# hku-mars/ImMesh

Measured on AMD Instinct MI355X. Metric: scans/sec (reg+mesh), 100k-pt scan into 10M-voxel map, higher is better.
Workload: dtype f64

## Files before the change

### immesh_amd/csrc/c_api.cpp

```cpp
#include "host_ctx.hpp"
#include "imu_host.hpp"
#include <cmath>
#include <new>

#define RP_ABORTED 1
static thread_local std::string g_create_error;
thread_local KProf* g_kprof = nullptr;



extern "C" {

void immesh_default_config(immesh_config* c) {
    std::memset(c, 0, sizeof(*c));
    c->voxel_size = 0.5; c->max_layer = 2;
    for (int i = 0; i < 5; i++) c->layer_init[i] = 5;
    c->max_points_size = 100; c->planer_threshold = 0.01; c->dept_err = 0.02; c->beam_err = 0.05; c->calib_laser = 0;
    c->sigma_num = 3.0; c->max_iter = 4;
    c->extR[0] = c->extR[4] = c->extR[8] = 1.0;
    c->extT[0] = 0.04165; c->extT[1] = 0.02326; c->extT[2] = -0.0284;
    c->mesh_min_spacing = 0.1; c->mesh_voxel = 0.4; c->mesh_region = 10.0; c->mesh_append_budget = 10000;
}

const char* immesh_create_error(void) { return g_create_error.c_str(); }
// ... 413 lines not shown

struct IngestOpts {
    int mode = 0;
    hipEvent_t after_point_var = nullptr;
    const ScanParams* spd = nullptr;
    const float* d_raw = nullptr; float* world = nullptr; int n_raw = 0;
    bool defer_tail = false;
    bool prep_done = false;
};
static int map_ingest_device(immesh_ctx* c, const float* d_pts, int64_t n, const imh::State& st, const IngestOpts& o) {
    ScanParams sp;
    make_scan_params(c, st, st.cov, sp);
    hipStream_t s = c->stream;
    if (o.mode == 0) {
        if (!o.prep_done) {
            if (c->tail_deferred) { launch_map_update_tail(s, c->map, c->d_counters_host); c->tail_deferred = false; }
            c->map.upd_seq++;
            c->map.touched = c->d_touched;
            launch_point_var(s, c->map, sp, o.spd, d_pts, (int)n, 3, o.mode, c->d_ptdata, c->d_key_a, c->d_slot, c->d_idx_a, o.d_raw, o.world, o.n_raw);
            if (o.world) { c->ev_inputs_cur = mesh_record_ready(c); c->inputs_seq = 0; }
            else if (o.after_point_var) { HIPCHK(c, hipEventRecord(o.after_point_var, s)); c->ev_inputs_cur = o.after_point_var; c->inputs_seq = 0; }
        }
        launch_replay_lists(s, c->map, c->d_idx_a, c->d_key_a, c->d_ptdata, (int)n, c->d_stats, c->d_counters_host, c->d_idx_b, c->d_idx_c, c->d_slot_s, c->reg_dbg, !o.defer_tail,
                            o.prep_done ? (unsigned long long*)(c->d_epi + 2) : nullptr, o.prep_done ? c->d_epi_flag_host : nullptr, c->epi_seq, c->knobs.fused_wgs, c->knobs.list_div);
        c->tail_deferred = o.defer_tail;
        return 0;
    }
    launch_point_var(s, c->map, sp, nullptr, d_pts, (int)n, 3, o.mode, c->d_ptdata, c->d_key_a, c->d_slot, nullptr);
    launch_iota(s, c->d_idx_a, (int)n);
    sort_pairs_u32(s, c->d_sort_temp, c->sort_temp_bytes, c->d_slot, c->d_slot_s, c->d_idx_a, c->d_idx_c, (int)n, 32);
    launch_segment_heads(s, c->d_slot_s, (int)n, c->d_seg_start, c->d_nseg);
    launch_replay(s, c->map, c->d_slot_s, c->d_idx_c, c->d_ptdata, (int)n, c->d_seg_start, c->d_nseg, (int)n, o.mode, c->d_stats);
    HIPCHK(c, hipMemcpyAsync(c->h_counters, c->map.counters, 16 * sizeof(int32_t), hipMemcpyDeviceToHost, s));
    return 0;
}

static int map_ingest_entry(immesh_ctx* c, const float* pts, int64_t n, const double* state, int mode) {
    if (!c || !pts || n <= 0 || n > c->cap_scan || !state) { if (c) c->err = "bad arguments"; return IMMESH_E_INVAL; }
    (void)hipSetDevice(c->cfg.device);
    ProfBind _pb(c);
    if (mode == 0) c->ds_gate_ok = false;
    if (const int s_rc = settle(c)) return s_rc;
    const void* d_pts;
    int rc = resolve_input(c, pts, (size_t)n * 12, c->d_pts_down, &d_pts);
    if (rc) return rc;
    imh::State st;
    imh::load_state(state, st);
// ... 300 lines not shown
```

### immesh_amd/csrc/host_knobs.hpp

```cpp
#pragma once
#include <hip/hip_runtime.h>
#include <algorithm>
#include <cstdlib>
#include <cstring>
#include <string>

struct Knobs {
    bool debug = false;
    bool debug_waits = false;
    std::string trace_file;
    int split_general = -1;
    bool no_priority = false;
    int mesh_cus = 0;
    int rp_blocks = 0;
    bool rp_force_abort = false;
    bool match_seq = false;
    bool host_ekf = false;
    bool serial_safe = false;
    bool serial_order = false;
    bool ds_radix = false;
    bool ds_no_gate = false;
    bool no_graph = false;
    int split_mode = 2;
    int mesh_room = 0;
    bool no_pipeline = false;
    int tri_stream = 1;
    int fused_wgs = 768;
    int list_div = 0;
    int mesh_grid_div = 1;

    static Knobs from_env(int mesh_npar) {
        auto on = [](const char* name) { return getenv(name) != nullptr; };
        auto num = [](const char* name, int unset) { const char* e = getenv(name); return e ? atoi(e) : unset; };
        Knobs k;
        k.debug = on("IMMESH_DEBUG"); k.debug_waits = on("IMMESH_DEBUG_WAITS");
        if (const char* e = getenv("IMMESH_TRACE_FILE")) k.trace_file = e;
        if (on("IMMESH_SPLIT_GENERAL")) k.split_general = num("IMMESH_SPLIT_GENERAL", 0);
        k.no_priority = on("IMMESH_NO_PRIORITY");
        k.mesh_cus = num("IMMESH_MESH_CUS", 0); if (k.mesh_cus < 8 || k.mesh_cus >= 1024) k.mesh_cus = 0;
        if (on("IMMESH_RP_BLOCKS")) k.rp_blocks = std::max(1, num("IMMESH_RP_BLOCKS", 0));
        k.rp_force_abort = on("IMMESH_RP_FORCE_ABORT"); k.match_seq = on("IMMESH_MATCH_SEQ"); k.host_ekf = on("IMMESH_HOST_EKF");
        k.serial_safe = on("IMMESH_SERIAL_SAFE"); k.serial_order = on("IMMESH_SERIAL_ORDER");
        k.ds_radix = on("IMMESH_DS_RADIX"); k.ds_no_gate = on("IMMESH_DS_NO_GATE");
        k.no_graph = on("IMMESH_NO_GRAPH");
        k.split_mode = on("IMMESH_NO_SPLIT") ? 0 : 2;
        if (on("IMMESH_SPLIT")) k.split_mode = num("IMMESH_SPLIT", 0) == 0 ? 0 : 1;
        if (on("IMMESH_MESH_ROOM")) k.mesh_room = std::min(std::max(num("IMMESH_MESH_ROOM", 0), 1), mesh_npar);
        k.no_pipeline = on("IMMESH_NO_PIPELINE");
        k.tri_stream = num("IMMESH_TRI_STREAM", 1);
        { const int v = num("IMMESH_FUSED_WGS", 0); k.fused_wgs = v >= 32 ? v : 768; }
        { const int v = num("IMMESH_LIST_DIV", 0); k.list_div = v >= 4 ? v : 0; }
        k.mesh_grid_div = std::max(1, num("IMMESH_MESH_GRID_DIV", 1));
        return k;
    }

    hipError_t make_stream(hipStream_t* s, int priority, bool maskable) const {
        if (!maskable || !mesh_cus) return hipStreamCreateWithPriority(s, hipStreamNonBlocking, priority);
        uint32_t mask[32];
        std::memset(mask, 0, sizeof(mask));
        for (int i = 0; i < mesh_cus; i++) mask[i >> 5] |= 1u << (i & 31);
        return hipExtStreamCreateWithCUMask(s, 32, mask);
    }
};
```

### immesh_amd/csrc/kernels.hpp

```cpp
#pragma once
#include <hip/hip_runtime.h>
#include <stdint.h>

struct RegMapDev;

struct ScanParams {
    double R[9], t[3];
    double extR[9], extT[3];
    double RextR[9];
    double rot_var[9], t_var[9];
    double dvar_beam;
    double dvar_calib;
    double sigma_num;
    float dept_err;
    int calib_laser;
    unsigned long long* dbg;
};

struct PlaneRecDev {
    long long key[3];
    int layer, path, is_plane, n_points, update_enable, new_points;
    float radius, min_eig, d, pad;
    double center[3], normal[3], plane_var[36];
};
// ... 37 lines not shown
};
static_assert(REG_OUT_COV + 18 * 18 == REG_OUT_PASSES && REG_OUT_TICKET == REG_OUT_DOUBLES - 1, "registration result block layout");

void launch_residual(hipStream_t s, const RegMapDev& m, const RegIterArgs& a, RegState* rs, const float* pts, int n, double* partials, unsigned int* done_counter,
                     double* out48, double* reg_out, double ticket, int8_t* o_match, int32_t* o_node, float* o_dis, double* o_rinv, double* o_normal);
#define RP_SLOT_DOUBLES (64 * 128 * 32)
#define RP_SLOT_SENTINEL 0x7FF8DEADBEEF0001ull
struct RpEpilogue {
    int enabled, n_raw;
    double* pt_data; unsigned long long* sort_key; uint32_t* slot_out; int32_t* pt_next;
    const float* raw; float* world;
};
#define RP_TAIL_WORD (63 * 128 * 32)
#define RP_ABORT_WORD (62 * 128 * 32)
void launch_residual_persistent(hipStream_t s, const RegMapDev& m, const RegIterArgs& a, RegState* rs, const float* pts, int n, double* slots, double* slots_next,
                                int32_t* host_counters, double* reg_out, double ticket, int8_t* o_match, int32_t* o_node, float* o_dis, double* o_rinv, double* o_normal,
                                const RpEpilogue& ep, int max_blocks);
int residual_persistent_resident_blocks(int device);
void launch_ekf_step(hipStream_t s, const RegIterArgs& a, RegState* rs, const double* sums48, double* reg_out, double ticket);
void launch_point_var(hipStream_t s, const RegMapDev& m, const ScanParams& sp, const ScanParams* spd, const float* pts, int n, int stride, int mode, double* pt_data,
                      unsigned long long* sort_key, uint32_t* slot, int32_t* pt_next, const float* raw_xyzi = nullptr, float* world_xyzi = nullptr, int n_raw = 0);
void launch_replay_lists(hipStream_t s, const RegMapDev& m, const int32_t* pt_next, const unsigned long long* sort_key, const double* pt_data, int n,
                         int64_t* stats, int32_t* host_counters, int32_t* big_idx, int32_t* big_order, uint32_t* general_list, unsigned long long* dbg, bool with_tail, unsigned long long* flag_dev, unsigned long long* flag_host, unsigned long long flag_seq,
                         int fused_wgs, int list_div_knob);
void launch_map_update_tail(hipStream_t s, const RegMapDev& m, int32_t* host_counters);
void launch_segment_heads(hipStream_t s, const uint32_t* sorted_slot, int n, int32_t* seg_start, int32_t* nseg);
void launch_replay(hipStream_t s, const RegMapDev& m, const uint32_t* sorted_slot, const int32_t* sorted_idx, const double* pt_data, int n,
                   const int32_t* seg_start, const int32_t* nseg, int max_segments, int mode, int64_t* stats);
void launch_dump_planes(hipStream_t s, const RegMapDev& m, PlaneRecDev* out, long long cap, unsigned long long* count);
void launch_fill_u64(hipStream_t s, unsigned long long* p, unsigned long long v, size_t n);
void launch_iota(hipStream_t s, int32_t* p, int n);
void launch_unpack_strided(hipStream_t s, const void* src, int n, int stride_bytes, int intensity_off_bytes, float* out);

void launch_ds_minmax(hipStream_t s, const float* pts, int n, int stride, float inv, int* mm);
void launch_ds_index(hipStream_t s, const float* pts, int n, int stride, float inv, const int* mm, unsigned long long* keys, int32_t* vals);
void launch_ds_heads(hipStream_t s, const unsigned long long* keys_sorted, int n, int32_t* flags);
void launch_ds_centroid(hipStream_t s, const float* pts, int n, int stride, const unsigned long long* keys_sorted, const int32_t* idx_sorted, const int32_t* rank,
                        float* out, int32_t* n_out);
void launch_decode_livox_count(hipStream_t s, const uint8_t* w, int n, int n_scans, int32_t* counted);
void launch_decode_livox_keep(hipStream_t s, const uint8_t* w, int n, int n_scans, int filter, double blind_sqr, const int32_t* valid_excl, int32_t* keep);
void launch_decode_livox_emit(hipStream_t s, const uint8_t* w, int n, const int32_t* keep, const int32_t* pos, float* out, int32_t* n_out);
void launch_decode_velodyne_keep(hipStream_t s, const uint8_t* d, int n, int step, int ox, int oy, int oz, float q_lo, float q_hi, int32_t* keep);
void launch_decode_velodyne_emit(hipStream_t s, const uint8_t* d, int n, int step, int ox, int oy, int oz, int oi, const int32_t* keep, const int32_t* pos, float* out,
                                 int32_t* n_out);
void launch_undistort_keys(hipStream_t s, const float* pts5, int n, uint32_t* key, int32_t* idx);
void launch_undistort(hipStream_t s, const float* pts5, const int32_t* order, int n, const double* poses, int n_poses, const double* fe, float* out_xyzi);
struct DsDyn { const float* pts; float* out; int32_t n, stride; float inv; int32_t pad; const int32_t* gate_word; int32_t gate_val, gate_pad; };
// ... 16 lines not shown
```

### immesh_amd/csrc/reg_kernels.hip

```cpp
#include <algorithm>
#include <cstdlib>
#include "regmap.hpp"
#include "kernels.hpp"
#include "prof.hpp"

using namespace imd;

struct PlaneRegs { double n[3], c[3], pv[21]; float d, radius; };
struct BestMatch { int node; int layer; double prob; bool ok; PlaneRegs P; };

IMD double plane_sigma(const double* pv, const double* J) {
    double tmp[6];
#pragma unroll
    for (int c = 0; c < 6; c++) {
        double s = 0;
#pragma unroll
        for (int r = 0; r < 6; r++) s += J[r] * pv[(r <= c) ? sym21_index(r, c) : sym21_index(c, r)];
        tmp[c] = s;
    }
    double sig = 0;
#pragma unroll
    for (int c = 0; c < 6; c++) sig += tmp[c] * J[c];
    return sig;
}
// ... 1305 lines not shown
        const double Umin[3] = {sel3(imin, f.U[0], f.U[1], f.U[2]), sel3(imin, f.U[3], f.U[4], f.U[5]), sel3(imin, f.U[6], f.U[7], f.U[8])};
        if (lane < 21) {
            double v = 0;
#pragma unroll
            for (int k = 0; k < 21; k++) if (lane == k) v = pv[k];
            nr.p_var[lane] = v;
        }
        if (lane == 0) {
            const double evmin = sel3(imin, f.ev[0], f.ev[1], f.ev[2]);
            const double evmax = sel3(f.imax, f.ev[0], f.ev[1], f.ev[2]);
#pragma unroll
            for (int k = 0; k < 3; k++) { nr.p_center[k] = f.c[k]; nr.p_normal[k] = Umin[k]; }
            nr.min_eig = (float)evmin;
            nr.radius = (float)sqrt(evmax);
            nr.d = (float)(-(Umin[0] * f.c[0] + Umin[1] * f.c[1] + Umin[2] * f.c[2]));
        }
    } else if (lane == 0) {
#pragma unroll
        for (int k = 0; k < 3; k++) { nr.p_center[k] = f.c[k]; nr.p_normal[k] = 0.0; }
        nr.radius = 0.f;
    }
}

__device__ __noinline__ bool wave_init_plane(const RegMapDev& m, int nd, int n, const WaveCtx& w) {
    __builtin_amdgcn_fence(__ATOMIC_ACQUIRE, "workgroup");
    if (w.lane == 0 && w.stats) { atomicAdd((unsigned long long*)&w.stats[0], 1ull); atomicAdd((unsigned long long*)&w.stats[1], (unsigned long long)n); }
    PlaneFit f;
    double pv[21];
    const int lane = w.lane;
    if (n <= 128) {
        double P0[9], P1[9];
#pragma unroll
        for (int k = 0; k < 9; k++) { P0[k] = 0; P1[k] = 0; }
        if (lane < n) { const double* q = node_point_ptr(m, nd, lane);
#pragma unroll
            for (int k = 0; k < 9; k++) P0[k] = q[k]; }
        if (lane + 64 < n) { const double* q = node_point_ptr(m, nd, lane + 64);
#pragma unroll
            for (int k = 0; k < 9; k++) P1[k] = q[k]; }
        auto fe = [&](auto&& fn) __attribute__((always_inline)) { if (lane < n) fn(P0); if (lane + 64 < n) fn(P1); };
        fit_eigen(fe, n, m.planer_threshold, f);
        if (f.planar) fit_plane_var(fe, n, f, pv);
    } else {
        auto fe = [&](auto&& fn) __attribute__((always_inline)) {
            for (int i = lane; i < n; i += 64) {
                const double* q = node_point_ptr(m, nd, i);
                double P[9];
#pragma unroll
                for (int k = 0; k < 9; k++) P[k] = q[k];
                fn(P);
            }
        };
        fit_eigen(fe, n, m.planer_threshold, f);
        if (f.planar) fit_plane_var(fe, n, f, pv);
    }
    fit_store(m.nodes[nd], f, pv, lane);
    return f.planar;
}

__device__ bool wave_push_point(const RegMapDev& m, int nd, int n, const double* src, const WaveCtx& w) {
    int ok = 1;
    if (w.lane == 0 && (n % IM_CHUNK_PTS) == 0) ok = node_ensure_chunk(m, nd, n / IM_CHUNK_PTS) ? 1 : 0;
    ok = __shfl(ok, 0, 64);
    if (!ok) return false;
    __builtin_amdgcn_fence(__ATOMIC_RELEASE, "workgroup");
    __builtin_amdgcn_fence(__ATOMIC_ACQUIRE, "workgroup");
    if (w.lane < IM_PT_DOUBLES) {
        double* dst = node_point_ptr(m, nd, n);
        dst[w.lane] = src[w.lane];
    }
    __builtin_amdgcn_fence(__ATOMIC_RELEASE, "workgroup");
    return true;
}

IMD int octant_of(const double* q, const double* center) {
    return 4 * (q[0] > center[0] ? 1 : 0) + 2 * (q[1] > center[1] ? 1 : 0) + (q[2] > center[2] ? 1 : 0);
}
IMD int make_child(const RegMapDev& m, int nd, int oct) {
    const float ql = m.nodes[nd].quarter;
    const int xyz[3] = {(oct >> 2) & 1, (oct >> 1) & 1, oct & 1};
    double c[3];
#pragma unroll
    for (int k = 0; k < 3; k++) c[k] = m.nodes[nd].center[k] + (double)((float)(2 * xyz[k] - 1) * ql);
    const int layer = m.nodes[nd].layer + 1;
    const int child = node_alloc(m, layer, c, ql / 2, m.nodes[nd].key, m.nodes[nd].path | (oct << (3 * (layer - 1))));
    m.nodes[nd].child[oct] = child;
    return child;
}

__device__ void wave_init_octo_tree(const RegMapDev& m, int node, int* stack, const WaveCtx& w) {
    int sp = 0;
    if (w.lane == 0) stack[0] = node;
    sp = 1;
    while (sp > 0) {
        __builtin_amdgcn_fence(__ATOMIC_ACQUIRE, "workgroup");
        const int nd = __shfl(stack[sp - 1], 0, 64);
        sp--;
        const int n = m.nodes[nd].npts;
        const bool planar = wave_init_plane(m, nd, n, w);
        const int layer = m.nodes[nd].layer;
        if (w.lane == 0) {
            const int f0 = m.nodes[nd].flags;
            int f = f0 | NF_INIT;
            f = planar ? (f | NF_PLANE) : (f & ~NF_PLANE);
            node_set_flags(m, w.root, nd, f0, f, w.shared);
            m.nodes[nd].newpts = 0;
        }
        if (planar || layer >= m.max_layer) continue;
        const double ctr[3] = {m.nodes[nd].center[0], m.nodes[nd].center[1], m.nodes[nd].center[2]};
        int child_id[8], child_n[8];
#pragma unroll
        for (int k = 0; k < 8; k++) { child_id[k] = m.nodes[nd].child[k]; child_n[k] = child_id[k] >= 0 ? m.nodes[child_id[k]].npts : 0; }
        for (int base = 0; base < n; base += 64) {
            const int i = base + w.lane;
            const double* q = (i < n) ? node_point_ptr(m, nd, i) : nullptr;
            const int oct = (i < n) ? octant_of(q, ctr) : -1;
#pragma unroll
            for (int k = 0; k < 8; k++) {
                const unsigned long long mask = __ballot(oct == k);
                if (mask == 0) continue;
                const int cnt = __popcll(mask);
                int cid = child_id[k];
// ... 15 lines not shown
#pragma unroll
                    for (int e = 0; e < IM_PT_DOUBLES; e++) dst[e] = q[e];
                }
                child_n[k] += cnt;
            }
        }
        __builtin_amdgcn_fence(__ATOMIC_RELEASE, "workgroup");
        if (w.lane == 0) {
#pragma unroll
            for (int k = 0; k < 8; k++)
                if (child_id[k] >= 0) { m.nodes[child_id[k]].npts = child_n[k]; m.nodes[child_id[k]].newpts = child_n[k]; }
            node_free_points(m, nd);
        }
#pragma unroll
        for (int k = 7; k >= 0; k--)
            if (child_id[k] >= 0 && child_n[k] > m.init_size[min(layer + 1, 4)]) {
                if (w.lane == 0) stack[sp] = child_id[k];
                sp++;
            }
        __builtin_amdgcn_fence(__ATOMIC_RELEASE, "workgroup");
    }
}

__device__ void wave_update_point(const RegMapDev& m, int root, const double* src, int* stack, const WaveCtx& w) {
    int nd = root;
    for (int depth = 0; depth < 8; depth++) {
        __builtin_amdgcn_fence(__ATOMIC_ACQUIRE, "workgroup");
        const int flags = m.nodes[nd].flags;
        const int layer = m.nodes[nd].layer;
        const int n = m.nodes[nd].npts;
        if (!(flags & NF_INIT)) {
            if (!wave_push_point(m, nd, n, src, w)) return;
            if (w.lane == 0) { m.nodes[nd].npts = n + 1; m.nodes[nd].newpts = m.nodes[nd].newpts + 1; }
            __builtin_amdgcn_fence(__ATOMIC_RELEASE, "workgroup");
            if (n + 1 > m.init_size[min(layer, 4)]) wave_init_octo_tree(m, nd, stack, w);
            return;
        }
        if (flags & NF_PLANE) {
            if (!(flags & NF_UPDATE_EN)) return;
            if (!wave_push_point(m, nd, n, src, w)) return;
            int newp = m.nodes[nd].newpts + 1;
            if (w.lane == 0) m.nodes[nd].npts = n + 1;
            __builtin_amdgcn_fence(__ATOMIC_RELEASE, "workgroup");
            if (newp > 5) {
                const bool planar = wave_init_plane(m, nd, n + 1, w);
                if (w.lane == 0) node_set_flags(m, w.root, nd, flags, planar ? (flags | NF_PLANE) : (flags & ~NF_PLANE), w.shared);
                newp = 0;
            }
            if (w.lane == 0) {
                m.nodes[nd].newpts = newp;
                if (n + 1 >= m.max_points_size) {
                    m.nodes[nd].flags = m.nodes[nd].flags & ~NF_UPDATE_EN;
                    node_free_points(m, nd);
                    m.nodes[nd].newpts = 0;
                }
            }
            __builtin_amdgcn_fence(__ATOMIC_RELEASE, "workgroup");
            return;
        }
        if (layer < m.max_layer) {
            int child;
            if (w.lane == 0) {
                if (n != 0) node_free_points(m, nd);
                const double ctr[3] = {m.nodes[nd].center[0], m.nodes[nd].center[1], m.nodes[nd].center[2]};
                const int oct = octant_of(src, ctr);
                child = m.nodes[nd].child[oct];
                if (child < 0) child = make_child(m, nd, oct);
            }
            __builtin_amdgcn_fence(__ATOMIC_RELEASE, "workgroup");
            child = __shfl(child, 0, 64);
            if (child < 0) return;
            nd = child;
            continue;
        }
        if (!(flags & NF_UPDATE_EN)) return;
        if (!wave_push_point(m, nd, n, src, w)) return;
        int newp = m.nodes[nd].newpts + 1;
        if (w.lane == 0) m.nodes[nd].npts = n + 1;
        __builtin_amdgcn_fence(__ATOMIC_RELEASE, "workgroup");
        if (newp > 5) {
            const bool planar = wave_init_plane(m, nd, n + 1, w);
            if (w.lane == 0) node_set_flags(m, w.root, nd, flags, planar ? (flags | NF_PLANE) : (flags & ~NF_PLANE), w.shared);
            newp = 0;
        }
        if (w.lane == 0) {
            m.nodes[nd].newpts = newp;
            if (n + 1 > IM_G_MAX_POINTS) { m.nodes[nd].flags = m.nodes[nd].flags & ~NF_UPDATE_EN; node_free_points(m, nd); }
        }
        __builtin_amdgcn_fence(__ATOMIC_RELEASE, "workgroup");
        return;
    }
}

__device__ int wave_replay_planar_root(const RegMapDev& m, const int root, const int* order, const int cnt, const double* __restrict__ pt_data, const WaveCtx& w) {
    NodeRec& nd = m.nodes[root];
    int flags = nd.flags;
    const int layer = nd.layer;
    int npts = nd.npts, newp = nd.newpts;
    const int want = NF_INIT | NF_PLANE | NF_UPDATE_EN;
    if (layer == 0 && (flags & want) == (NF_INIT | NF_PLANE)) return cnt;
    if ((flags & want) != want || layer != 0 || npts + cnt > IM_INLINE_CHUNKS * IM_CHUNK_PTS) return 0;
    int chunks[IM_INLINE_CHUNKS];
#pragma unroll
    for (int k = 0; k < IM_INLINE_CHUNKS; k++) chunks[k] = nd.chunks[k];
    auto chunk_of = [&](int ci) { int c = chunks[0];
#pragma unroll
        for (int k = 1; k < IM_INLINE_CHUNKS; k++) { const int ck = chunks[k]; c = (ci == k) ? ck : c; }
        return c; };
    double s1[3] = {0, 0, 0}, s2[3] = {0, 0, 0};
    const bool will_refit = newp + cnt > 5;
    if (will_refit) {
        for (int i = w.lane; i < npts; i += 64) {
            const double* q = m.chunk_data + ((size_t)chunk_of(i / IM_CHUNK_PTS) * IM_CHUNK_PTS + (i % IM_CHUNK_PTS)) * IM_PT_DOUBLES;
#pragma unroll
            for (int a = 0; a < 3; a++) { const double v = q[a]; s1[a] += v; s2[a] += v * v; }
        }
// ... 24 lines not shown
            if (c < 0) { write_header(); return j; }
#pragma unroll
            for (int k = 0; k < IM_INLINE_CHUNKS; k++) if (ci == k) chunks[k] = c;
        }
        const double pv = w.lane < IM_PT_DOUBLES ? src[w.lane] : 0.0;
        if (w.lane < IM_PT_DOUBLES) m.chunk_data[((size_t)chunk_of(ci) * IM_CHUNK_PTS + (npts % IM_CHUNK_PTS)) * IM_PT_DOUBLES + w.lane] = pv;
        if (will_refit) {
#pragma unroll
            for (int a = 0; a < 3; a++) { const double v = __shfl(pv, a, 64); s1[a] += v; s2[a] += v * v; }
        }
        npts++; newp++; header_dirty = true;
        if (newp > 5) {
            n_ref++; n_ref_pts += npts;
            const double dn = (double)npts;
            double vmin = 1e300, mag = 0;
#pragma unroll
            for (int a = 0; a < 3; a++) { const double mu = s1[a] / dn; const double v = s2[a] / dn - mu * mu; vmin = fmin(vmin, v); mag += s2[a] / dn; }
            const double err = 1e-7 + 1e-12 * mag;
            newp = 0;
            if (vmin + err < (double)m.planer_threshold) last_refit_n = npts;
            else {
                write_header();
                last_refit_n = 0;
                const bool planar = wave_init_plane(m, root, npts, wq);
                if (!planar) {
                    if (w.lane == 0) node_set_flags(m, w.root, root, flags, flags & ~NF_PLANE);
                    __builtin_amdgcn_fence(__ATOMIC_RELEASE, "workgroup");
                    flags &= ~NF_PLANE;
                    if (npts >= m.max_points_size) {
                        flags &= ~NF_UPDATE_EN;
                        write_header();
                        if (w.lane == 0) { node_free_points(m, root); nd.newpts = 0; }
                        __builtin_amdgcn_fence(__ATOMIC_RELEASE, "workgroup");
                        npts = 0; newp = 0;
                    }
                    j++;
                    break;
                }
            }
        }
        if (npts >= m.max_points_size) {
            if (last_refit_n) { write_header(); (void)wave_init_plane(m, root, last_refit_n, wq); last_refit_n = 0; }
            flags &= ~NF_UPDATE_EN;
            write_header();
            if (w.lane == 0) { node_free_points(m, root); nd.newpts = 0; }
            __builtin_amdgcn_fence(__ATOMIC_RELEASE, "workgroup");
            npts = 0; newp = 0;
            j++;
            break;
        }
    }
    if (header_dirty) write_header();
    if (last_refit_n) (void)wave_init_plane(m, root, last_refit_n, wq);
    if (w.lane == 0 && w.stats && n_ref) { atomicAdd((unsigned long long*)&w.stats[0], (unsigned long long)n_ref); atomicAdd((unsigned long long*)&w.stats[1], (unsigned long long)n_ref_pts); }
    return j;
}

__device__ int wave_replay_planar_node(const RegMapDev& m, const int node, const int* order, const int cnt, const double* __restrict__ pt_data, const WaveCtx& w) {
    NodeRec& nd = m.nodes[node];
    int flags = nd.flags;
    const int want = NF_INIT | NF_PLANE | NF_UPDATE_EN;
    if ((flags & want) == (NF_INIT | NF_PLANE)) return cnt;
    if ((flags & want) != want) return 0;
    int npts = nd.npts, newp = nd.newpts;
    double s1[3] = {0, 0, 0}, s2[3] = {0, 0, 0};
    const bool will_refit = newp + cnt > 5;
    if (will_refit) {
        for (int i = w.lane; i < npts; i += 64) {
            const double* q = node_point_ptr(m, node, i);
#pragma unroll
            for (int a = 0; a < 3; a++) { const double v = q[a]; s1[a] += v; s2[a] += v * v; }
        }
#pragma unroll
        for (int a = 0; a < 3; a++) { s1[a] = wave_sum(s1[a]); s2[a] = wave_sum(s2[a]); }
    }
    WaveCtx wq = w; wq.stats = nullptr;
    int last_refit_n = 0, n_ref = 0, j = 0;
    long long n_ref_pts = 0;
    auto write_counts = [&]() {
        if (w.lane == 0) { nd.npts = npts; nd.newpts = newp; }
        __builtin_amdgcn_fence(__ATOMIC_RELEASE, "workgroup");
        __builtin_amdgcn_fence(__ATOMIC_ACQUIRE, "workgroup");
    };
    for (; j < cnt; j++) {
        const double* src = pt_data + (size_t)order[j] * IM_PT_DOUBLES;
        if (!wave_push_point(m, node, npts, src, w)) { write_counts(); return j; }
        if (will_refit) {
            const double pv = w.lane < IM_PT_DOUBLES ? src[w.lane] : 0.0;
#pragma unroll
            for (int a = 0; a < 3; a++) { const double v = __shfl(pv, a, 64); s1[a] += v; s2[a] += v * v; }
        }
        npts++; newp++;
        if (newp > 5) {
            n_ref++; n_ref_pts += npts;
            const double dn = (double)npts;
            double vmin = 1e300, mag = 0;
#pragma unroll
            for (int a = 0; a < 3; a++) { const double mu = s1[a] / dn; const double v = s2[a] / dn - mu * mu; vmin = fmin(vmin, v); mag += s2[a] / dn; }
            const double err = 1e-7 + 1e-12 * mag;
            newp = 0;
            if (vmin + err < (double)m.planer_threshold) last_refit_n = npts;
            else {
                write_counts();
                last_refit_n = 0;
                const bool planar = wave_init_plane(m, node, npts, wq);
                if (!planar) {
                    if (w.lane == 0) node_set_flags(m, w.root, node, flags, flags & ~NF_PLANE, w.shared);
                    __builtin_amdgcn_fence(__ATOMIC_RELEASE, "workgroup");
                    flags &= ~NF_PLANE;
                    if (npts >= m.max_points_size) {
                        write_counts();
                        if (w.lane == 0) { nd.flags = nd.flags & ~NF_UPDATE_EN; node_free_points(m, node); nd.newpts = 0; }
                        __builtin_amdgcn_fence(__ATOMIC_RELEASE, "workgroup");
                        npts = 0; newp = 0;
                    }
                    j++;
                    break;
                }
            }
        }
        if (npts >= m.max_points_size) {
            write_counts();
            if (last_refit_n) { (void)wave_init_plane(m, node, last_refit_n, wq); last_refit_n = 0; }
            if (w.lane == 0) { nd.flags = nd.flags & ~NF_UPDATE_EN; node_free_points(m, node); nd.newpts = 0; }
            __builtin_amdgcn_fence(__ATOMIC_RELEASE, "workgroup");
            npts = 0; newp = 0;
            j++;
            if (w.lane == 0 && w.stats && n_ref) { atomicAdd((unsigned long long*)&w.stats[0], (unsigned long long)n_ref); atomicAdd((unsigned long long*)&w.stats[1], (unsigned long long)n_ref_pts); }
            return j;
        }
    }
    write_counts();
    if (last_refit_n) (void)wave_init_plane(m, node, last_refit_n, wq);
    if (w.lane == 0 && w.stats && n_ref) { atomicAdd((unsigned long long*)&w.stats[0], (unsigned long long)n_ref); atomicAdd((unsigned long long*)&w.stats[1], (unsigned long long)n_ref_pts); }
    return j;
}

__global__ __launch_bounds__(256) void replay_kernel(RegMapDev m, const uint32_t* __restrict__ sorted_slot, const int32_t* __restrict__ sorted_idx,
                                                      const double* __restrict__ pt_data, int n, const int32_t* __restrict__ seg_start,
                                                      const int32_t* __restrict__ nseg, int mode, int64_t* stats) {
    __shared__ int stacks[4][48];
    const int wv = threadIdx.x >> 6;
    const int seg = blockIdx.x * 4 + wv;
    if (seg >= *nseg) return;
    WaveCtx w; w.lane = threadIdx.x & 63; w.stats = stats;
    const int start = seg_start[seg];
    const uint32_t slot = sorted_slot[start];
    const int root = m.htab[slot].root;
    if (root < 0) return;
    w.root = root;
    if (mode == 0) {
        for (int j = start; j < n && sorted_slot[j] == slot; j++)
            wave_update_point(m, root, pt_data + (size_t)sorted_idx[j] * IM_PT_DOUBLES, stacks[wv], w);
    } else {
        int cnt = m.nodes[root].npts;
        for (int j = start; j < n && sorted_slot[j] == slot; j++) {
            if (!wave_push_point(m, root, cnt, pt_data + (size_t)sorted_idx[j] * IM_PT_DOUBLES, w)) return;
            cnt++;
        }
        if (w.lane == 0) { m.nodes[root].npts = cnt; m.nodes[root].newpts = cnt; }
        __builtin_amdgcn_fence(__ATOMIC_RELEASE, "workgroup");
        if (cnt > m.init_size[0]) wave_init_octo_tree(m, root, stacks[wv], w);
    }
}

#define RL_CAP 64
#define DBG_FUSED_OFF 64
#define DBG_FUSED_RECS 16384
#define DBG_RES_OFF (DBG_FUSED_OFF + DBG_FUSED_RECS * 8)
static_assert(DBG_RES_OFF + 8 * 512 * 8 == REG_DBG_WORDS, "the IMMESH_DEBUG buffer (kernels.hpp) holds the counters and both trace areas");
#define RF_PTS 128
__global__ __launch_bounds__(256, 3) void replay_fused_kernel(RegMapDev m, const int32_t* __restrict__ pt_next, const unsigned long long* __restrict__ sort_key,
                                                            const double* __restrict__ pt_data, int64_t* stats, uint32_t* __restrict__ general_list,
                                                            unsigned long long* __restrict__ dbg, unsigned long long* flag_dev, unsigned long long* flag_host,
                                                            unsigned long long flag_seq) {
    if (flag_dev && blockIdx.x == 0 && threadIdx.x == 0) {
        __hip_atomic_store(flag_dev, flag_seq, __ATOMIC_RELAXED, __HIP_MEMORY_SCOPE_AGENT);
        __hip_atomic_store(flag_host, flag_seq, __ATOMIC_RELAXED, __HIP_MEMORY_SCOPE_SYSTEM);
    }
    __shared__ unsigned long long skey[4][RL_CAP];
    __shared__ int sidx[4][RL_CAP];
    __shared__ int order[4][RL_CAP];
    __builtin_amdgcn_s_setprio(REG_UPD_PRIO);
    const int wv = threadIdx.x >> 6, lane = threadIdx.x & 63;
    const int t_first = blockIdx.x * 4 + wv, t_stride = gridDim.x * 4;
    uint32_t slot_first = m.touched[2 * (size_t)t_first];
    int root_first = (int)m.touched[2 * (size_t)t_first + 1];
    const int n_touched = m.counters[7];
#define FDBG(k) do { if (dbg) { const unsigned long long _t = __builtin_readcyclecounter(); if (tr) ((unsigned int*)tr)[4 + (k)] = (unsigned int)(_t - tprev); tprev = _t; } } while (0)
#define FEND(state, nref) do { if (tr) { tr[1] = __builtin_amdgcn_s_memrealtime(); tr[7] = (unsigned long long)((unsigned)cnt | ((unsigned)(nref) << 8) | ((unsigned)(state) << 16)); } } while (0)
    auto process = [&](const int t, const uint32_t slot, int root) __attribute__((always_inline)) {
    unsigned long long* const tr = (dbg && lane == 0 && t < DBG_FUSED_RECS) ? dbg + DBG_FUSED_OFF + (size_t)t * 8 : nullptr;
    unsigned long long tprev = dbg ? __builtin_readcyclecounter() : 0;
    if (tr) { tr[0] = __builtin_amdgcn_s_memrealtime(); tr[2] = tr[3] = tr[4] = tr[5] = tr[6] = tr[7] = 0; }
    if (root < 0) root = m.htab[slot].root;
    if (root < 0) return;
    FDBG(0);
    NodeRec& nd = m.nodes[root];
    const int flags = nd.flags, layer = nd.layer;
    const int npts = nd.npts, newp = nd.newpts;
    if (dbg) { asm volatile("s_waitcnt vmcnt(0)" ::: "memory"); FDBG(1); }
    int chunks[IM_INLINE_CHUNKS];
#pragma unroll
    for (int k = 0; k < IM_INLINE_CHUNKS; k++) chunks[k] = nd.chunks[k];
    if (dbg) { asm volatile("s_waitcnt vmcnt(0)" ::: "memory"); FDBG(2); }
    int cnt = 0;
    int ihead = (int)(unsigned int)(m.slot_head[slot] & 0xFFFFFFFFull);
    if (dbg) { asm volatile("s_waitcnt vmcnt(0)" ::: "memory"); FDBG(3); }
    for (int i = ihead; i >= 0; i = pt_next[i]) {
        if (cnt < RL_CAP && lane == 0) { skey[wv][cnt] = sort_key[i]; sidx[wv][cnt] = i; }
        cnt++;
    }
    FDBG(4);
    const int want = NF_INIT | NF_PLANE | NF_UPDATE_EN;
// ... 81 lines not shown
                    for (int k = 0; k < 9; k++) d[k] = P0[k]; }
                if (q1 >= npts && q1 < ntot) { double* d = m.chunk_data + ((size_t)chunk_of(q1 >> 4) * IM_CHUNK_PTS + (q1 & 15)) * IM_PT_DOUBLES;
#pragma unroll
                    for (int k = 0; k < 9; k++) d[k] = P1[k]; }
            }
            if (lane == 0) {
                nd.npts = ntot; nd.newpts = (newp + cnt) % 6;
#pragma unroll
                for (int k = 0; k < IM_INLINE_CHUNKS; k++) nd.chunks[k] = chunks[k];
                if (n_ref) { int64_t* sh = stats + 16 + (size_t)(t & 63) * 16; atomicAdd((unsigned long long*)&sh[0], (unsigned long long)n_ref); atomicAdd((unsigned long long*)&sh[1], (unsigned long long)n_ref_pts); }
            }
            FDBG(8);
            if (n_ref > 0) {
                double pv[21];
                auto fe = [&](auto&& fn) __attribute__((always_inline)) { if (lane < n_last) fn(P0); if (lane + 64 < n_last) fn(P1); };
                fit_plane_var(fe, n_last, fit, pv);
                fit_store(nd, fit, pv, lane);
            }
            FDBG(9);
            FEND(2, n_ref);
            return;
        }
    }
    if (lane == 0) general_list[atomicAdd(&m.counters[10], 1)] = slot;
    FEND(3, 0);
    };
    for (int t = t_first; t < n_touched; t += t_stride) {
        if (t != t_first) { slot_first = m.touched[2 * (size_t)t]; root_first = (int)m.touched[2 * (size_t)t + 1]; }
        process(t, slot_first, root_first);
    }
#undef FDBG
#undef FEND
}

__device__ bool replay_split_root(const RegMapDev& m, const int root, const int* order, const int cnt, const double* __restrict__ pt_data, const WaveCtx& w);
__device__ bool replay_split_leaves(const RegMapDev& m, const int root, const int* order, const int cnt, const double* __restrict__ pt_data, const WaveCtx& w, int* s_key, int* s_first);
__global__ __launch_bounds__(256) void replay_list_kernel(RegMapDev m, const int32_t* __restrict__ pt_next, const unsigned long long* __restrict__ sort_key,
                                                           const double* __restrict__ pt_data, int64_t* stats, int32_t* __restrict__ big_idx, int32_t* __restrict__ big_order,
                                                           unsigned long long* __restrict__ dbg, const uint32_t* __restrict__ work, const int32_t* __restrict__ n_work) {
    __shared__ unsigned long long skey[4][RL_CAP];
    __shared__ int sidx[4][RL_CAP];
    __shared__ int order[4][RL_CAP];
    __shared__ int stacks[4][48];
    __builtin_amdgcn_s_setprio(REG_UPD_PRIO);
    const int wv = threadIdx.x >> 6;
    const int nw = *n_work;
    WaveCtx w; w.lane = threadIdx.x & 63; w.stats = stats;
    for (int t = blockIdx.x * 4 + wv; t < nw; t += gridDim.x * 4) {
        const uint32_t slot = work[t];
        const int root = m.htab[slot].root;
        if (root < 0) continue;
        w.root = root;
// ... 261 lines not shown
    const int nb = std::max(1, std::min((n + 255) / 256, std::min(max_blocks, RP_MAX_BLOCKS)));
    if (!(a.pad & 4) && m.cap_nodes < (1 << 26)) KLAUNCH(residual_persistent_kernel<true>, dim3(nb + 1), dim3(256), 0, s, m, a, rs, pts, n, slots, slots_next, a.max_iter * RP_MAX_BLOCKS * RES_NR, host_counters, reg_out, ticket, o_match, o_node,
            o_dis, o_rinv, o_normal, ep);
    else KLAUNCH(residual_persistent_kernel<false>, dim3(nb + 1), dim3(256), 0, s, m, a, rs, pts, n, slots, slots_next, a.max_iter * RP_MAX_BLOCKS * RES_NR, host_counters, reg_out, ticket, o_match, o_node,
            o_dis, o_rinv, o_normal, ep);
}
int residual_persistent_resident_blocks(int device) {
    int per_cu = 0, cus = 0;
    if (hipOccupancyMaxActiveBlocksPerMultiprocessor(&per_cu, residual_persistent_kernel<true>, 256, 0) != hipSuccess) { (void)hipGetLastError(); per_cu = 1; }
    if (hipDeviceGetAttribute(&cus, hipDeviceAttributeMultiprocessorCount, device) != hipSuccess) { (void)hipGetLastError(); cus = 0; }
    return std::max(1, per_cu) * cus;
}
void launch_ekf_step(hipStream_t s, const RegIterArgs& a, RegState* rs, const double* sums48, double* reg_out, double ticket) {
    KLAUNCH(ekf_step_kernel, dim3(1), dim3(64), 0, s, a, rs, sums48, reg_out, ticket);
}
void launch_point_var(hipStream_t s, const RegMapDev& m, const ScanParams& sp, const ScanParams* spd, const float* pts, int n, int stride, int mode, double* pt_data,
                      unsigned long long* sort_key, uint32_t* slot, int32_t* pt_next, const float* raw_xyzi, float* world_xyzi, int n_raw) {
    const int nb_pv = (n + 255) / 256, nb_x = raw_xyzi ? (n_raw + 255) / 256 : 0;
    KLAUNCH(point_var_kernel, dim3(nb_pv + nb_x), dim3(256), 0, s, m, sp, spd, pts, n, stride, mode, pt_data, sort_key, slot, pt_next, (const float4*)raw_xyzi,
            (float4*)world_xyzi, n_raw, nb_pv);
}
void launch_replay_lists(hipStream_t s, const RegMapDev& m, const int32_t* pt_next, const unsigned long long* sort_key, const double* pt_data, int n,
                         int64_t* stats, int32_t* host_counters, int32_t* big_idx, int32_t* big_order, uint32_t* general_list, unsigned long long* dbg, bool with_tail,
                         unsigned long long* flag_dev, unsigned long long* flag_host, unsigned long long flag_seq, int fused_wgs, int list_div_knob) {
    KLAUNCH(replay_fused_kernel, dim3(std::min((n + 3) / 4, fused_wgs)), dim3(256), 0, s, m, pt_next, sort_key, pt_data, stats, general_list, dbg, flag_dev, flag_host, flag_seq);
    const int list_div = list_div_knob ? list_div_knob : (m.split_general ? 32 : 128);
    const int nb_list = std::min(std::max((n + list_div - 1) / list_div, 32), 4096);
    KLAUNCH(replay_list_kernel, dim3(nb_list), dim3(256), 0, s, m, pt_next, sort_key, pt_data, stats, big_idx, big_order, dbg, (const uint32_t*)general_list,
            (const int32_t*)(m.counters + 10));
    if (m.split_general) KLAUNCH(replay_sub_kernel, dim3(std::min(std::max((n + 15) / 16, 32), 2048)), dim3(256), 0, s, m, pt_data, stats);
    if (with_tail) KLAUNCH(merge_free_tail_kernel, dim3(1), dim3(256), 0, s, m, host_counters);
}
void launch_map_update_tail(hipStream_t s, const RegMapDev& m, int32_t* host_counters) { KLAUNCH(merge_free_tail_kernel, dim3(1), dim3(256), 0, s, m, host_counters); }
void launch_segment_heads(hipStream_t s, const uint32_t* sorted_slot, int n, int32_t* seg_start, int32_t* nseg) {
    (void)hipMemsetAsync(nseg, 0, sizeof(int32_t), s);
    KLAUNCH(segment_heads_kernel, dim3((n + 255) / 256), dim3(256), 0, s, sorted_slot, n, seg_start, nseg);
}
void launch_replay(hipStream_t s, const RegMapDev& m, const uint32_t* sorted_slot, const int32_t* sorted_idx, const double* pt_data, int n,
                   const int32_t* seg_start, const int32_t* nseg, int max_segments, int mode, int64_t* stats) {
    KLAUNCH(replay_kernel, dim3((max_segments + 3) / 4), dim3(256), 0, s, m, sorted_slot, sorted_idx, pt_data, n, seg_start, nseg, mode, stats);
    KLAUNCH(merge_free_kernel, dim3(64), dim3(256), 0, s, m);
    KLAUNCH(merge_free_finish_kernel, dim3(1), dim3(1), 0, s, m);
}
void launch_dump_planes(hipStream_t s, const RegMapDev& m, PlaneRecDev* out, long long cap, unsigned long long* count) {
    (void)hipMemsetAsync(count, 0, sizeof(unsigned long long), s);
    KLAUNCH(dump_planes_kernel, dim3(1024), dim3(256), 0, s, m, out, cap, count);
}
void launch_fill_u64(hipStream_t s, unsigned long long* p, unsigned long long v, size_t n) {
    KLAUNCH(fill_u64_kernel, dim3(2048), dim3(256), 0, s, p, v, n);
}
void launch_iota(hipStream_t s, int32_t* p, int n) { KLAUNCH(iota_kernel, dim3((n + 255) / 256), dim3(256), 0, s, p, n); }
```

Measured before the change: 5920.

## Process general-path voxels in place within fused replay kernel instead of second launch

```diff
diff --git a/immesh_amd/csrc/c_api.cpp b/immesh_amd/csrc/c_api.cpp
--- a/immesh_amd/csrc/c_api.cpp
+++ b/immesh_amd/csrc/c_api.cpp
@@ -459,7 +459,7 @@
             else if (o.after_point_var) { HIPCHK(c, hipEventRecord(o.after_point_var, s)); c->ev_inputs_cur = o.after_point_var; c->inputs_seq = 0; }
         }
         launch_replay_lists(s, c->map, c->d_idx_a, c->d_key_a, c->d_ptdata, (int)n, c->d_stats, c->d_counters_host, c->d_idx_b, c->d_idx_c, c->d_slot_s, c->reg_dbg, !o.defer_tail,
-                            o.prep_done ? (unsigned long long*)(c->d_epi + 2) : nullptr, o.prep_done ? c->d_epi_flag_host : nullptr, c->epi_seq, c->knobs.fused_wgs, c->knobs.list_div);
+                            o.prep_done ? (unsigned long long*)(c->d_epi + 2) : nullptr, o.prep_done ? c->d_epi_flag_host : nullptr, c->epi_seq, c->knobs.fused_wgs, c->knobs.list_div, c->knobs.replay_two_launch);
         c->tail_deferred = o.defer_tail;
         return 0;
     }
diff --git a/immesh_amd/csrc/host_knobs.hpp b/immesh_amd/csrc/host_knobs.hpp
--- a/immesh_amd/csrc/host_knobs.hpp
+++ b/immesh_amd/csrc/host_knobs.hpp
@@ -27,6 +27,7 @@
     int tri_stream = 1;
     int fused_wgs = 768;
     int list_div = 0;
+    bool replay_two_launch = false;
     int mesh_grid_div = 1;
 
     static Knobs from_env(int mesh_npar) {
@@ -50,6 +51,7 @@
         k.tri_stream = num("IMMESH_TRI_STREAM", 1);
         { const int v = num("IMMESH_FUSED_WGS", 0); k.fused_wgs = v >= 32 ? v : 768; }
         { const int v = num("IMMESH_LIST_DIV", 0); k.list_div = v >= 4 ? v : 0; }
+        k.replay_two_launch = on("IMMESH_REPLAY_TWO_LAUNCH");
         k.mesh_grid_div = std::max(1, num("IMMESH_MESH_GRID_DIV", 1));
         return k;
     }
diff --git a/immesh_amd/csrc/kernels.hpp b/immesh_amd/csrc/kernels.hpp
--- a/immesh_amd/csrc/kernels.hpp
+++ b/immesh_amd/csrc/kernels.hpp
@@ -83,7 +83,7 @@
                       unsigned long long* sort_key, uint32_t* slot, int32_t* pt_next, const float* raw_xyzi = nullptr, float* world_xyzi = nullptr, int n_raw = 0);
 void launch_replay_lists(hipStream_t s, const RegMapDev& m, const int32_t* pt_next, const unsigned long long* sort_key, const double* pt_data, int n,
                          int64_t* stats, int32_t* host_counters, int32_t* big_idx, int32_t* big_order, uint32_t* general_list, unsigned long long* dbg, bool with_tail, unsigned long long* flag_dev, unsigned long long* flag_host, unsigned long long flag_seq,
-                         int fused_wgs, int list_div_knob);
+                         int fused_wgs, int list_div_knob, bool two_launch);
 void launch_map_update_tail(hipStream_t s, const RegMapDev& m, int32_t* host_counters);
 void launch_segment_heads(hipStream_t s, const uint32_t* sorted_slot, int n, int32_t* seg_start, int32_t* nseg);
 void launch_replay(hipStream_t s, const RegMapDev& m, const uint32_t* sorted_slot, const int32_t* sorted_idx, const double* pt_data, int n,
diff --git a/immesh_amd/csrc/reg_kernels.hip b/immesh_amd/csrc/reg_kernels.hip
--- a/immesh_amd/csrc/reg_kernels.hip
+++ b/immesh_amd/csrc/reg_kernels.hip
@@ -1351,6 +1351,7 @@
     }
 }
 
+template <int OWN = 0>
 __device__ __noinline__ bool wave_init_plane(const RegMapDev& m, int nd, int n, const WaveCtx& w) {
     __builtin_amdgcn_fence(__ATOMIC_ACQUIRE, "workgroup");
     if (w.lane == 0 && w.stats) { atomicAdd((unsigned long long*)&w.stats[0], 1ull); atomicAdd((unsigned long long*)&w.stats[1], (unsigned long long)n); }
@@ -1387,6 +1388,7 @@
     return f.planar;
 }
 
+template <int OWN = 0>
 __device__ bool wave_push_point(const RegMapDev& m, int nd, int n, const double* src, const WaveCtx& w) {
     int ok = 1;
     if (w.lane == 0 && (n % IM_CHUNK_PTS) == 0) ok = node_ensure_chunk(m, nd, n / IM_CHUNK_PTS) ? 1 : 0;
@@ -1417,6 +1419,7 @@
     return child;
 }
 
+template <int OWN = 0>
 __device__ void wave_init_octo_tree(const RegMapDev& m, int node, int* stack, const WaveCtx& w) {
     int sp = 0;
     if (w.lane == 0) stack[0] = node;
@@ -1426,7 +1429,7 @@
         const int nd = __shfl(stack[sp - 1], 0, 64);
         sp--;
         const int n = m.nodes[nd].npts;
-        const bool planar = wave_init_plane(m, nd, n, w);
+        const bool planar = wave_init_plane<OWN>(m, nd, n, w);
         const int layer = m.nodes[nd].layer;
         if (w.lane == 0) {
             const int f0 = m.nodes[nd].flags;
@@ -1488,6 +1491,7 @@
     }
 }
 
+template <int OWN = 0>
 __device__ void wave_update_point(const RegMapDev& m, int root, const double* src, int* stack, const WaveCtx& w) {
     int nd = root;
     for (int depth = 0; depth < 8; depth++) {
@@ -1496,20 +1500,20 @@
         const int layer = m.nodes[nd].layer;
         const int n = m.nodes[nd].npts;
         if (!(flags & NF_INIT)) {
-            if (!wave_push_point(m, nd, n, src, w)) return;
+            if (!wave_push_point<OWN>(m, nd, n, src, w)) return;
             if (w.lane == 0) { m.nodes[nd].npts = n + 1; m.nodes[nd].newpts = m.nodes[nd].newpts + 1; }
             __builtin_amdgcn_fence(__ATOMIC_RELEASE, "workgroup");
-            if (n + 1 > m.init_size[min(layer, 4)]) wave_init_octo_tree(m, nd, stack, w);
+            if (n + 1 > m.init_size[min(layer, 4)]) wave_init_octo_tree<OWN>(m, nd, stack, w);
             return;
         }
         if (flags & NF_PLANE) {
             if (!(flags & NF_UPDATE_EN)) return;
-            if (!wave_push_point(m, nd, n, src, w)) return;
+            if (!wave_push_point<OWN>(m, nd, n, src, w)) return;
             int newp = m.nodes[nd].newpts + 1;
             if (w.lane == 0) m.nodes[nd].npts = n + 1;
             __builtin_amdgcn_fence(__ATOMIC_RELEASE, "workgroup");
             if (newp > 5) {
-                const bool planar = wave_init_plane(m, nd, n + 1, w);
+                const bool planar = wave_init_plane<OWN>(m, nd, n + 1, w);
                 if (w.lane == 0) node_set_flags(m, w.root, nd, flags, planar ? (flags | NF_PLANE) : (flags & ~NF_PLANE), w.shared);
                 newp = 0;
             }
@@ -1540,12 +1544,12 @@
             continue;
         }
         if (!(flags & NF_UPDATE_EN)) return;
-        if (!wave_push_point(m, nd, n, src, w)) return;
+        if (!wave_push_point<OWN>(m, nd, n, src, w)) return;
         int newp = m.nodes[nd].newpts + 1;
         if (w.lane == 0) m.nodes[nd].npts = n + 1;
         __builtin_amdgcn_fence(__ATOMIC_RELEASE, "workgroup");
         if (newp > 5) {
-            const bool planar = wave_init_plane(m, nd, n + 1, w);
+            const bool planar = wave_init_plane<OWN>(m, nd, n + 1, w);
             if (w.lane == 0) node_set_flags(m, w.root, nd, flags, planar ? (flags | NF_PLANE) : (flags & ~NF_PLANE), w.shared);
             newp = 0;
         }
@@ -1558,6 +1562,7 @@
     }
 }
 
+template <int OWN = 0>
 __device__ int wave_replay_planar_root(const RegMapDev& m, const int root, const int* order, const int cnt, const double* __restrict__ pt_data, const WaveCtx& w) {
     NodeRec& nd = m.nodes[root];
     int flags = nd.flags;
@@ -1628,7 +1633,7 @@
             else {
                 write_header();
                 last_refit_n = 0;
-                const bool planar = wave_init_plane(m, root, npts, wq);
+                const bool planar = wave_init_plane<OWN>(m, root, npts, wq);
                 if (!planar) {
                     if (w.lane == 0) node_set_flags(m, w.root, root, flags, flags & ~NF_PLANE);
                     __builtin_amdgcn_fence(__ATOMIC_RELEASE, "workgroup");
@@ -1646,7 +1651,7 @@
             }
         }
         if (npts >= m.max_points_size) {
-            if (last_refit_n) { write_header(); (void)wave_init_plane(m, root, last_refit_n, wq); last_refit_n = 0; }
+            if (last_refit_n) { write_header(); (void)wave_init_plane<OWN>(m, root, last_refit_n, wq); last_refit_n = 0; }
             flags &= ~NF_UPDATE_EN;
             write_header();
             if (w.lane == 0) { node_free_points(m, root); nd.newpts = 0; }
@@ -1657,11 +1662,12 @@
         }
     }
     if (header_dirty) write_header();
-    if (last_refit_n) (void)wave_init_plane(m, root, last_refit_n, wq);
+    if (last_refit_n) (void)wave_init_plane<OWN>(m, root, last_refit_n, wq);
     if (w.lane == 0 && w.stats && n_ref) { atomicAdd((unsigned long long*)&w.stats[0], (unsigned long long)n_ref); atomicAdd((unsigned long long*)&w.stats[1], (unsigned long long)n_ref_pts); }
     return j;
 }
 
+template <int OWN = 0>
 __device__ int wave_replay_planar_node(const RegMapDev& m, const int node, const int* order, const int cnt, const double* __restrict__ pt_data, const WaveCtx& w) {
     NodeRec& nd = m.nodes[node];
     int flags = nd.flags;
@@ -1690,7 +1696,7 @@
     };
     for (; j < cnt; j++) {
         const double* src = pt_data + (size_t)order[j] * IM_PT_DOUBLES;
-        if (!wave_push_point(m, node, npts, src, w)) { write_counts(); return j; }
+        if (!wave_push_point<OWN>(m, node, npts, src, w)) { write_counts(); return j; }
         if (will_refit) {
             const double pv = w.lane < IM_PT_DOUBLES ? src[w.lane] : 0.0;
 #pragma unroll
@@ -1709,7 +1715,7 @@
             else {
                 write_counts();
                 last_refit_n = 0;
-                const bool planar = wave_init_plane(m, node, npts, wq);
+                const bool planar = wave_init_plane<OWN>(m, node, npts, wq);
                 if (!planar) {
                     if (w.lane == 0) node_set_flags(m, w.root, node, flags, flags & ~NF_PLANE, w.shared);
                     __builtin_amdgcn_fence(__ATOMIC_RELEASE, "workgroup");
@@ -1727,7 +1733,7 @@
         }
         if (npts >= m.max_points_size) {
             write_counts();
-            if (last_refit_n) { (void)wave_init_plane(m, node, last_refit_n, wq); last_refit_n = 0; }
+            if (last_refit_n) { (void)wave_init_plane<OWN>(m, node, last_refit_n, wq); last_refit_n = 0; }
             if (w.lane == 0) { nd.flags = nd.flags & ~NF_UPDATE_EN; node_free_points(m, node); nd.newpts = 0; }
             __builtin_amdgcn_fence(__ATOMIC_RELEASE, "workgroup");
             npts = 0; newp = 0;
@@ -1737,7 +1743,7 @@
         }
     }
     write_counts();
-    if (last_refit_n) (void)wave_init_plane(m, node, last_refit_n, wq);
+    if (last_refit_n) (void)wave_init_plane<OWN>(m, node, last_refit_n, wq);
     if (w.lane == 0 && w.stats && n_ref) { atomicAdd((unsigned long long*)&w.stats[0], (unsigned long long)n_ref); atomicAdd((unsigned long long*)&w.stats[1], (unsigned long long)n_ref_pts); }
     return j;
 }
@@ -1776,10 +1782,74 @@
 #define DBG_RES_OFF (DBG_FUSED_OFF + DBG_FUSED_RECS * 8)
 static_assert(DBG_RES_OFF + 8 * 512 * 8 == REG_DBG_WORDS, "the IMMESH_DEBUG buffer (kernels.hpp) holds the counters and both trace areas");
 #define RF_PTS 128
+__device__ __forceinline__ int replay_voxel_own(const RegMapDev& m, const uint32_t slot, const int32_t* __restrict__ pt_next, const unsigned long long* __restrict__ sort_key,
+                                             const double* __restrict__ pt_data, unsigned long long* skey, int* sidx, int* order, int* stack,
+                                             int32_t* __restrict__ big_idx, int32_t* __restrict__ big_order, const int lane, int64_t* stats, unsigned long long* __restrict__ dbg) {
+    const int root = m.htab[slot].root;
+    if (root < 0) return 0;
+    WaveCtx w; w.lane = lane; w.stats = stats; w.root = root;
+    const unsigned long long tdbg0 = dbg ? __builtin_readcyclecounter() : 0;
+    __builtin_amdgcn_wave_barrier();
+    const int ihead = (int)(unsigned int)(m.slot_head[slot] & 0xFFFFFFFFull);
+    int cnt = 0;
+    for (int i = ihead; i >= 0; i = pt_next[i]) {
+        if (cnt < RL_CAP && lane == 0) { skey[cnt] = sort_key[i]; sidx[cnt] = i; }
+        cnt++;
+    }
+    const int* ord = order;
+    if (cnt > RL_CAP) {
+        int base = 0;
+        if (lane == 0) base = atomicAdd(&m.counters[9], cnt);
+        base = __shfl(base, 0, 64);
+        if (lane == 0) { int k = 0; for (int i = ihead; i >= 0; i = pt_next[i]) big_idx[base + k++] = i; }
+        __builtin_amdgcn_fence(__ATOMIC_RELEASE, "agent");
+        __builtin_amdgcn_wave_barrier();
+        __builtin_amdgcn_fence(__ATOMIC_ACQUIRE, "agent");
+        for (int e = lane; e < cnt; e += 64) {
+            const int id = big_idx[base + e];
+            const unsigned long long k = sort_key[id];
+            int rank = 0;
+            for (int f = 0; f < cnt; f++) { const int idf = big_idx[base + f]; const unsigned long long kf = sort_key[idf]; rank += (kf < k || (kf == k && idf < id)) ? 1 : 0; }
+            big_order[base + rank] = id;
+        }
+        __builtin_amdgcn_fence(__ATOMIC_RELEASE, "agent");
+        __builtin_amdgcn_wave_barrier();
+        __builtin_amdgcn_fence(__ATOMIC_ACQUIRE, "agent");
+        ord = big_order + base;
+    } else {
+        __builtin_amdgcn_fence(__ATOMIC_RELEASE, "workgroup");
+        __builtin_amdgcn_wave_barrier();
+        __builtin_amdgcn_fence(__ATOMIC_ACQUIRE, "workgroup");
+        for (int e = lane; e < cnt; e += 64) {
+            const unsigned long long k = skey[e];
+            const int id = sidx[e];
+            int rank = 0;
+            for (int f = 0; f < cnt; f++) { const unsigned long long kf = skey[f]; rank += (kf < k || (kf == k && sidx[f] < id)) ? 1 : 0; }
+            order[rank] = id;
+        }
+        __builtin_amdgcn_fence(__ATOMIC_RELEASE, "workgroup");
+        __builtin_amdgcn_wave_barrier();
+        __builtin_amdgcn_fence(__ATOMIC_ACQUIRE, "workgroup");
+    }
+    const unsigned long long tdbg1 = dbg ? __builtin_readcyclecounter() : 0;
+    int jf = wave_replay_planar_root<1>(m, root, ord, cnt, pt_data, w);
+    if (jf == 0) jf = wave_replay_planar_node<1>(m, root, ord, cnt, pt_data, w);
+    for (int j = jf; j < cnt; j++) wave_update_point<1>(m, root, pt_data + (size_t)ord[j] * IM_PT_DOUBLES, stack, w);
+    if (dbg && lane == 0) {
+        const unsigned long long t2 = __builtin_readcyclecounter();
+        atomicMax(&dbg[jf == cnt ? 8 : 9], ((t2 - tdbg0) << 16) | (unsigned long long)cnt);
+        atomicAdd(&dbg[jf == cnt ? 10 : 11], t2 - tdbg1);
+        atomicAdd(&dbg[jf == cnt ? 12 : 13], 1ull);
+        atomicAdd(&dbg[14], tdbg1 - tdbg0);
+    }
+    return jf == cnt ? 4 : 5;
+}
+
+template <bool INPLACE>
 __global__ __launch_bounds__(256, 3) void replay_fused_kernel(RegMapDev m, const int32_t* __restrict__ pt_next, const unsigned long long* __restrict__ sort_key,
                                                             const double* __restrict__ pt_data, int64_t* stats, uint32_t* __restrict__ general_list,
                                                             unsigned long long* __restrict__ dbg, unsigned long long* flag_dev, unsigned long long* flag_host,
-                                                            unsigned long long flag_seq) {
+                                                            unsigned long long flag_seq, int32_t* __restrict__ big_idx, int32_t* __restrict__ big_order) {
     if (flag_dev && blockIdx.x == 0 && threadIdx.x == 0) {
         __hip_atomic_store(flag_dev, flag_seq, __ATOMIC_RELAXED, __HIP_MEMORY_SCOPE_AGENT);
         __hip_atomic_store(flag_host, flag_seq, __ATOMIC_RELAXED, __HIP_MEMORY_SCOPE_SYSTEM);
@@ -1787,6 +1857,7 @@
     __shared__ unsigned long long skey[4][RL_CAP];
     __shared__ int sidx[4][RL_CAP];
     __shared__ int order[4][RL_CAP];
+    __shared__ int stacks[4][48];
     __builtin_amdgcn_s_setprio(REG_UPD_PRIO);
     const int wv = threadIdx.x >> 6, lane = threadIdx.x & 63;
     const int t_first = blockIdx.x * 4 + wv, t_stride = gridDim.x * 4;
@@ -1795,7 +1866,8 @@
     const int n_touched = m.counters[7];
 #define FDBG(k) do { if (dbg) { const unsigned long long _t = __builtin_readcyclecounter(); if (tr) ((unsigned int*)tr)[4 + (k)] = (unsigned int)(_t - tprev); tprev = _t; } } while (0)
 #define FEND(state, nref) do { if (tr) { tr[1] = __builtin_amdgcn_s_memrealtime(); tr[7] = (unsigned long long)((unsigned)cnt | ((unsigned)(nref) << 8) | ((unsigned)(state) << 16)); } } while (0)
-    auto process = [&](const int t, const uint32_t slot, int root) __attribute__((always_inline)) {
+    unsigned long long deferred = 0;
+    auto process = [&](const int t, const int k, const uint32_t slot, int root) __attribute__((always_inline)) {
     unsigned long long* const tr = (dbg && lane == 0 && t < DBG_FUSED_RECS) ? dbg + DBG_FUSED_OFF + (size_t)t * 8 : nullptr;
     unsigned long long tprev = dbg ? __builtin_readcyclecounter() : 0;
     if (tr) { tr[0] = __builtin_amdgcn_s_memrealtime(); tr[2] = tr[3] = tr[4] = tr[5] = tr[6] = tr[7] = 0; }
@@ -1923,12 +1995,26 @@
             return;
         }
     }
-    if (lane == 0) general_list[atomicAdd(&m.counters[10], 1)] = slot;
+    if (INPLACE) deferred |= 1ull << k;
+    else if (lane == 0) general_list[atomicAdd(&m.counters[10], 1)] = slot;
     FEND(3, 0);
     };
-    for (int t = t_first; t < n_touched; t += t_stride) {
+    int k = 0;
+    for (int t = t_first; t < n_touched && (!INPLACE || k < 64); t += t_stride, k++) {
         if (t != t_first) { slot_first = m.touched[2 * (size_t)t]; root_first = (int)m.touched[2 * (size_t)t + 1]; }
-        process(t, slot_first, root_first);
+        process(t, k, slot_first, root_first);
+    }
+    if (INPLACE) {
+        const RegMapDev& mk = *(const RegMapDev*)__builtin_amdgcn_kernarg_segment_ptr();
+        k = 0;
+        for (int t = t_first; t < n_touched; t += t_stride, k++) {
+            if (k < 64 && !((deferred >> k) & 1ull)) continue;
+            unsigned long long* const tr = (dbg && lane == 0 && t < DBG_FUSED_RECS) ? dbg + DBG_FUSED_OFF + (size_t)t * 8 : nullptr;
+            if (tr) tr[0] = __builtin_amdgcn_s_memrealtime();
+            const int st = replay_voxel_own(mk, m.touched[2 * (size_t)t], pt_next, sort_key, pt_data, skey[wv], sidx[wv], order[wv], stacks[wv], big_idx, big_order, lane,
+                                            stats + 16 + (size_t)(t & 63) * 16, dbg);
+            if (tr) { tr[1] = __builtin_amdgcn_s_memrealtime(); tr[7] = (tr[7] & 0xFFFFull) | ((unsigned long long)st << 16); }
+        }
     }
 #undef FDBG
 #undef FEND
@@ -2236,12 +2322,18 @@
 }
 void launch_replay_lists(hipStream_t s, const RegMapDev& m, const int32_t* pt_next, const unsigned long long* sort_key, const double* pt_data, int n,
                          int64_t* stats, int32_t* host_counters, int32_t* big_idx, int32_t* big_order, uint32_t* general_list, unsigned long long* dbg, bool with_tail,
-                         unsigned long long* flag_dev, unsigned long long* flag_host, unsigned long long flag_seq, int fused_wgs, int list_div_knob) {
-    KLAUNCH(replay_fused_kernel, dim3(std::min((n + 3) / 4, fused_wgs)), dim3(256), 0, s, m, pt_next, sort_key, pt_data, stats, general_list, dbg, flag_dev, flag_host, flag_seq);
+                         unsigned long long* flag_dev, unsigned long long* flag_host, unsigned long long flag_seq, int fused_wgs, int list_div_knob, bool two_launch) {
+    const bool inplace = !m.split_general && !two_launch;
+    if (inplace) KLAUNCH(replay_fused_kernel<true>, dim3(std::min((n + 3) / 4, fused_wgs)), dim3(256), 0, s, m, pt_next, sort_key, pt_data, stats, general_list, dbg, flag_dev, flag_host,
+            flag_seq, big_idx, big_order);
+    else KLAUNCH(replay_fused_kernel<false>, dim3(std::min((n + 3) / 4, fused_wgs)), dim3(256), 0, s, m, pt_next, sort_key, pt_data, stats, general_list, dbg, flag_dev, flag_host,
+            flag_seq, big_idx, big_order);
+    if (!inplace) {
     const int list_div = list_div_knob ? list_div_knob : (m.split_general ? 32 : 128);
     const int nb_list = std::min(std::max((n + list_div - 1) / list_div, 32), 4096);
     KLAUNCH(replay_list_kernel, dim3(nb_list), dim3(256), 0, s, m, pt_next, sort_key, pt_data, stats, big_idx, big_order, dbg, (const uint32_t*)general_list,
             (const int32_t*)(m.counters + 10));
+    }
     if (m.split_general) KLAUNCH(replay_sub_kernel, dim3(std::min(std::max((n + 15) / 16, 32), 2048)), dim3(256), 0, s, m, pt_data, stats);
     if (with_tail) KLAUNCH(merge_free_tail_kernel, dim3(1), dim3(256), 0, s, m, host_counters);
 }
```

After: 5822. 1.7% lower.
